# rafaelsoStanford/State_Policy_DiffusionModel

Hardware: AMD Instinct MI355X
Metric: denoise-steps/sec (B=4096, horizon=32) (higher is better)
Workload: dtype f32 (split-fp16 MFMA operands, fp32 accumulate)

## Files before the change

### state_policy_diffusionmodel_amd/csrc/device_utils.h

```cpp
#pragma once
#include <hip/hip_runtime.h>
#include "kernels.h"

namespace spdm {

__device__ __forceinline__ void sample_mean_rstd(const StatsRef& st, int b, float& mean, float& rstd) {
    const long long r0 = (long long)b * st.HW;
    const int first = (int)(r0 / st.m_tile);
    const int last = (int)((r0 + st.HW - 1) / st.m_tile);
    const int n = (last - first + 1) * st.n_tiles;
    const double* p = st.p + (size_t)b * st.slots * 2;
    double s1 = 0.0, s2 = 0.0;
    for (int i = 0; i < n; ++i) { s1 += p[2 * i]; s2 += p[2 * i + 1]; }
    const double m = s1 * st.inv_count;
    double var = s2 * st.inv_count - m * m;
    if (var < 0.0) var = 0.0;
    mean = (float)m;
    rstd = (float)(1.0 / sqrt(var + 1e-5));
}

__device__ __forceinline__ float sum_xor32(float v) {
    const unsigned u = __builtin_bit_cast(unsigned, v);
    const auto r = __builtin_amdgcn_permlane32_swap(u, u, false, false);
    return __builtin_bit_cast(float, (unsigned)r[0]) + __builtin_bit_cast(float, (unsigned)r[1]);
}
__device__ __forceinline__ float max_xor32(float v) {
    const unsigned u = __builtin_bit_cast(unsigned, v);
    const auto r = __builtin_amdgcn_permlane32_swap(u, u, false, false);
    return fmaxf(__builtin_bit_cast(float, (unsigned)r[0]), __builtin_bit_cast(float, (unsigned)r[1]));
}
__device__ __forceinline__ float sum_xor16(float v) {
    const unsigned u = __builtin_bit_cast(unsigned, v);
    const auto r = __builtin_amdgcn_permlane16_swap(u, u, false, false);
    return __builtin_bit_cast(float, (unsigned)r[0]) + __builtin_bit_cast(float, (unsigned)r[1]);
}
__device__ __forceinline__ double sum_xor32_f64(double v) {
    const unsigned long long u = __builtin_bit_cast(unsigned long long, v);
    const unsigned lo = (unsigned)u, hi = (unsigned)(u >> 32);
    const auto rl = __builtin_amdgcn_permlane32_swap(lo, lo, false, false);
    const auto rh = __builtin_amdgcn_permlane32_swap(hi, hi, false, false);
    const double a = __builtin_bit_cast(double, ((unsigned long long)(unsigned)rh[0] << 32) | (unsigned)rl[0]);
    const double b = __builtin_bit_cast(double, ((unsigned long long)(unsigned)rh[1] << 32) | (unsigned)rl[1]);
    return a + b;
// ... 154 lines not shown
```

### state_policy_diffusionmodel_amd/csrc/kernels.h

```cpp
#pragma once
#include <hip/hip_runtime.h>
#include <stdint.h>
#include <mutex>
#include <set>
#include <utility>
#include <vector>

namespace spdm {

inline hipError_t allow_full_lds(const void* kern) {
    static std::mutex mu;
    static std::set<std::pair<int, const void*>> done;
    int dev = 0;
    hipError_t e = hipGetDevice(&dev);
    if (e != hipSuccess) return e;
    std::lock_guard<std::mutex> lk(mu);
    if (done.count({dev, kern})) return hipSuccess;
    e = hipFuncSetAttribute(kern, hipFuncAttributeMaxDynamicSharedMemorySize, (int)(160 * 1024));
    if (e == hipSuccess) done.insert({dev, kern});
    return e;
}

struct StatsRef {
    const double* p;
// ... 2 lines not shown
    int n_tiles;
    int HW;
    double inv_count;
};

__host__ __device__ inline int stats_slots(int HW, int m_tile, int n_tiles) {
    return ((HW + m_tile - 2) / m_tile + 1) * n_tiles;
}

enum : unsigned {
    SW_NO_WIDE = 1u << 0, SW_NO_WIDE128 = 1u << 1, SW_NO_W2 = 1u << 2, SW_NO_T512 = 1u << 3, SW_T512 = 1u << 4,
    SW_T3_BIG = 1u << 5, SW_NO_SMALL_TPI3 = 1u << 6, SW_WIDE_N64_2X2 = 1u << 7, SW_NO_SA_FUSED = 1u << 8,
    SW_NO_SA_TAIL = 1u << 9, SW_ATTN_VALU = 1u << 10, SW_SA_NO_WLDS = 1u << 11, SW_NO_FILM_FOLD = 1u << 12,
    SW_NO_GRAPH = 1u << 13, SW_NO_SPLITK = 1u << 14, SW_ARENA_TRACE = 1u << 15, SW_NO_WIDE_PIPE = 1u << 16, SW_NO_SKINNY = 1u << 17, SW_DEEP = 1u << 18,
    SW_NO_FILM_LOCAL = 1u << 19, SW_NO_FUSED_SRC = 1u << 20, SW_FILM_LOCAL = 1u << 21, SW_PIN_GEOMETRY = 1u << 22, SW_NO_WP4 = 1u << 23, SW_G2 = 1u << 24, SW_NO_WP8 = 1u << 25, SW_NO_SA_HEAD = 1u << 26, SW_SA_HEAD = 1u << 27, SW_NO_REG64 = 1u << 28,
    SW_NO_SA_CROP = 1u << 29, SW_NO_SA_OUTC = 1u << 30,
};
struct SwitchName { const char* env; unsigned bit; };
inline const SwitchName* switch_table(int* n) {
    static const SwitchName t[] = {
        {"SPDM_NO_WIDE", SW_NO_WIDE}, {"SPDM_NO_WIDE128", SW_NO_WIDE128}, {"SPDM_NO_W2", SW_NO_W2}, {"SPDM_NO_T512", SW_NO_T512},
        {"SPDM_T512", SW_T512}, {"SPDM_T3_BIG", SW_T3_BIG}, {"SPDM_NO_SMALL_TPI3", SW_NO_SMALL_TPI3},
        {"SPDM_WIDE_N64_2X2", SW_WIDE_N64_2X2}, {"SPDM_NO_SA_FUSED", SW_NO_SA_FUSED}, {"SPDM_NO_SA_TAIL", SW_NO_SA_TAIL},
        {"SPDM_ATTN_VALU", SW_ATTN_VALU}, {"SPDM_SA_NO_WLDS", SW_SA_NO_WLDS}, {"SPDM_NO_FILM_FOLD", SW_NO_FILM_FOLD},
        {"SPDM_NO_GRAPH", SW_NO_GRAPH}, {"SPDM_NO_SPLITK", SW_NO_SPLITK}, {"SPDM_ARENA_TRACE", SW_ARENA_TRACE}, {"SPDM_NO_WIDE_PIPE", SW_NO_WIDE_PIPE}, {"SPDM_NO_SKINNY", SW_NO_SKINNY}, {"SPDM_DEEP", SW_DEEP},
        {"SPDM_NO_FILM_LOCAL", SW_NO_FILM_LOCAL}, {"SPDM_NO_FUSED_SRC", SW_NO_FUSED_SRC},
        {"SPDM_FILM_LOCAL", SW_FILM_LOCAL}, {"SPDM_PIN_GEOMETRY", SW_PIN_GEOMETRY},
        {"SPDM_NO_WP4", SW_NO_WP4}, {"SPDM_G2", SW_G2}, {"SPDM_NO_WP8", SW_NO_WP8},
        {"SPDM_NO_SA_HEAD", SW_NO_SA_HEAD}, {"SPDM_SA_HEAD", SW_SA_HEAD}, {"SPDM_NO_REG64", SW_NO_REG64},
        {"SPDM_NO_SA_CROP", SW_NO_SA_CROP}, {"SPDM_NO_SA_OUTC", SW_NO_SA_OUTC}};
    *n = (int)(sizeof(t) / sizeof(t[0]));
    return t;
}
unsigned switches_from_env();
int spdm_tune(int idx, int dflt);

enum { PRO_NONE = 0, PRO_GN = 1, PRO_GN_GELU = 2, PRO_POOL = 3, PRO_UPCAT = 4 };
enum { EPI_STATS = 0, EPI_BIAS = 1, EPI_BIAS_GELU = 2, EPI_BIAS_RESID = 3, EPI_PLAIN = 4 };

enum { ROUTE_GEMM = 0, ROUTE_SKINNY = 1, ROUTE_REG = 2, ROUTE_WIDE = 3 };
enum { VAR_PLAIN = 0, VAR_W2 = 1, VAR_WP4 = 2, VAR_WP8 = 3, VAR_PIPE = 4, VAR_G2 = 5 };
struct GemmRoute { int kernel, variant, m_tile, n_tile; };

struct GemmArgs {
    const float* src;  int src_ld;
// ... 154 lines not shown
struct SaCrop { int H0, D, Wp, lh, lw; const float* outc_w; float outc_b; float* eps; };
bool sa_crop_supported(int L, int C, int H0, int D);
hipError_t launch_sa_fused64(const float* x, float* out, int B, int L, const float* ln1_g, const float* ln1_b,
                             const float* ln2_g, const float* ln2_b, const void* const w_hl[8], const float* bqkv,
                             const float* bo, const float* b1, const float* b2, const float* ab, unsigned sw, hipStream_t s,
                             const FilmSpec* fs = nullptr, const SaCrop* crop = nullptr);

bool sa_tail_supported(int C, unsigned sw);
hipError_t launch_sa_tail(int C, const float* o, const float* x, float* out, int rows, const float* wf_o, const float* wf_1,
                          const float* wf_2, const float* b_o, const float* b_1, const float* b_2, const float* ln_g,
                          const float* ln_b, const float* ab, int L, hipStream_t s, const FilmSpec* fs = nullptr);
bool sa_tail_film_local(int C, int L);
bool sa_head_supported(int C, int L, unsigned sw);
hipError_t launch_sa_head(int C, const float* x, float* att, int rows, const float* wf_in, const float* b_in, const float* ln_g,
                          const float* ln_b, const float* ab, int L, hipStream_t s, const FilmSpec* fs = nullptr);
hipError_t launch_sa_qkv(int C, const float* x, float* qkv, int rows, const float* wf_in, const float* b_in, const float* ln_g,
                         const float* ln_b, const float* ab, int L, hipStream_t s, const FilmSpec* fs = nullptr);

}
```

### state_policy_diffusionmodel_amd/csrc/sa_tail.hip

```cpp
#include <algorithm>
#include <cstdlib>

#include "device_utils.h"

namespace spdm {

namespace {

typedef float tf32x4 __attribute__((ext_vector_type(4)));
typedef float tf32x2 __attribute__((ext_vector_type(2)));
typedef _Float16 tf16x8 __attribute__((ext_vector_type(8)));
typedef _Float16 tf16x2 __attribute__((ext_vector_type(2)));

constexpr float T_ACT_SCALE = 16.0f;
constexpr float T_DESCALE = 1.0f / 2048.0f;
constexpr int T_LDK = 36;
template <int C> struct TailShape {
    static_assert(C == 128 || C == 256, "C = 128 or 256");
    static constexpr int TM = 8192 / C;
    static constexpr int WM = TM / 32, WN = 4 / WM;
    static constexpr int NCH = C / 32;
    static constexpr int TPR = C / 4, RPP = 256 / TPR;
    static constexpr int NP = TM / RPP;
};

struct SaTailArgs {
    const float* o;
// ... 1 lines not shown
    float* out;
    int M;
    const float *wf_o, *wf_1, *wf_2;
    const float *b_o, *b_1, *b_2, *ln_g, *ln_b;
    const float* ab; int L;
    FilmSpec fs;
};

__device__ __forceinline__ tf32x2 tsplit2_plain(float a, float b) {
    const float xa = a * T_ACT_SCALE, xb = b * T_ACT_SCALE;
    const _Float16 ha = (_Float16)xa, hb = (_Float16)xb;
    const tf16x2 h = {ha, hb};
    const tf16x2 l = {(_Float16)(xa - (float)ha), (_Float16)(xb - (float)hb)};
    return tf32x2{__builtin_bit_cast(float, h), __builtin_bit_cast(float, l)};
}
#define TAIL_SPLIT2 tsplit2
__device__ __forceinline__ tf32x2 tsplit2(float a, float b) {
    unsigned h, l;
    split_pair_f16(a * T_ACT_SCALE, b * T_ACT_SCALE, h, l);
    return tf32x2{__builtin_bit_cast(float, h), __builtin_bit_cast(float, l)};
}
template <int TPR>
__device__ __forceinline__ float trow_sum(float v) {
    static_assert(TPR == 32 || TPR == 64, "rows of 32 or 64 lanes");
    v = sum_xor16(row16_sum_dpp(v));
    if (TPR == 64) v = sum_xor32(v);
    return v;
}

template <int C>
__device__ __forceinline__ void tail_film_fold(tf32x4 (&v)[8], const float* __restrict__ ab, int L, int m0, int M, int cq, int srow0) {
// ... 30 lines not shown
#pragma unroll
        for (int i = 0; i < 8; ++i) {
            const float* ab_ = abl + (size_t)(min(m0 + S::RPP * i + srow0, M - 1) / L - b_first) * 2 * C + cq * 4;
            v[i] = v[i] * *reinterpret_cast<const tf32x4*>(ab_) + *reinterpret_cast<const tf32x4*>(ab_ + C);
        }
    }
}

#ifdef SPDM_DIAG_TAIL
__device__ unsigned long long g_tail_stamps[64];
#define TAIL_STAMP(k_) if (blockIdx.x == 0 && threadIdx.x == 0) { asm volatile("s_waitcnt vmcnt(0) lgkmcnt(0)" ::: "memory"); g_tail_stamps[(C == 256 ? 16 : 0) + (k_)] = __builtin_amdgcn_s_memrealtime(); }
#else
#define TAIL_STAMP(k_)
#endif

template <int C>
__global__ __launch_bounds__(256, 2) void sa_tail_kernel(const SaTailArgs a) {
    TAIL_STAMP(0)
    using S = TailShape<C>;
    constexpr int T_C = C, T_M = S::TM, NCH = S::NCH, RPP = S::RPP, TPR = S::TPR;
    constexpr int RT = 2, CT = 4;
    constexpr int NP = S::NP;
    extern __shared__ __attribute__((aligned(16))) float smem[];
    const int tid = threadIdx.x, lane = tid & 63;
    const int wave = __builtin_amdgcn_readfirstlane(tid >> 6);
    const int wm = wave / S::WN, wn = wave % S::WN, l16 = lane & 15, kg = lane >> 4;
    const int M = a.M;
    const int m0 = blockIdx.x * T_M;

    float* Abuf = smem;
    float* otile = smem;

    const int c16 = tid % TPR, srow0 = tid / TPR;
    const int aoff0 = (wm * 32 + l16) * T_LDK + kg * 4;

    const size_t wlane = ((size_t)(wn * CT) * 2) * 256 + lane * 4;
    constexpr size_t WCHUNK = (size_t)(C / 16) * 2 * 256;
    tf16x8 fb[2][CT][2], fa[2][2];
#define TAIL_LOAD_B(slot_, w_, kc_)                                                                  \
    {                                                                                                \
        const float* p_ = (w_) + wlane + (size_t)(kc_) * WCHUNK;                                     \
        _Pragma("unroll") for (int c_ = 0; c_ < CT; ++c_) {                                         \
            fb[slot_][c_][0] = *reinterpret_cast<const tf16x8*>(p_ + c_ * 512);                      \
            fb[slot_][c_][1] = *reinterpret_cast<const tf16x8*>(p_ + c_ * 512 + 256);                \
        }                                                                                            \
    }
#define TAIL_LOAD_FA(slot_, kc_, rt_)                                                                \
    {                                                                                                \
        const float* p_ = Abuf + ((kc_) * T_M + (rt_) * 16) * T_LDK + aoff0;                         \
        fa[slot_][0] = *reinterpret_cast<const tf16x8*>(p_);                                         \
        fa[slot_][1] = *reinterpret_cast<const tf16x8*>(p_ + 16);                                    \
    }
#define TAIL_WRITE_SLAB(v_)                                                                          \
    _Pragma("unroll") for (int i_ = 0; i_ < NP; ++i_) {                                             \
        const tf32x2 p0_ = TAIL_SPLIT2(v_[i_].x, v_[i_].y), p1_ = TAIL_SPLIT2(v_[i_].z, v_[i_].w);   \
        float* rowp_ = Abuf + ((c16 >> 3) * T_M + RPP * i_ + srow0) * T_LDK;                         \
        *reinterpret_cast<tf32x2*>(rowp_ + (c16 & 7) * 2) = tf32x2{p0_.x, p1_.x};                    \
        *reinterpret_cast<tf32x2*>(rowp_ + 16 + (c16 & 7) * 2) = tf32x2{p0_.y, p1_.y};               \
    }
#define TAIL_GEMM(w_, wnext_)                                                                        \
    {                                                                                                \
        _Pragma("unroll") for (int rt_ = 0; rt_ < RT; ++rt_)                                        \
            _Pragma("unroll") for (int ct_ = 0; ct_ < CT; ++ct_) acc[rt_][ct_] = tf32x4{0.f, 0.f, 0.f, 0.f}; \
        TAIL_LOAD_FA(0, 0, 0)                                                                        \
        _Pragma("unroll") for (int kc = 0; kc < NCH; ++kc) {                                        \
            if (kc + 1 < NCH) { TAIL_LOAD_B((kc + 1) & 1, w_, kc + 1) } else { TAIL_LOAD_B(0, wnext_, 0) } \
            _Pragma("unroll") for (int rt = 0; rt < RT; ++rt) {                                     \
                if (rt + 1 < RT) { TAIL_LOAD_FA((rt + 1) & 1, kc, rt + 1) }                          \
                else if (kc + 1 < NCH) { TAIL_LOAD_FA(0, kc + 1, 0) }                                \
                __builtin_amdgcn_sched_barrier(0);                                                   \
// ... 16 lines not shown
                _Pragma("unroll") for (int j_ = 0; j_ < 4; ++j_)                                    \
                    otile[(wm * 32 + rt_ * 16 + 4 * kg + j_) * T_C + col_] = acc[rt_][ct_][j_] * T_DESCALE; \
            }                                                                                        \
        __syncthreads();                                                                             \
    }

    TAIL_LOAD_B(0, a.wf_o, 0)
    float* abl = smem + NCH * T_M * T_LDK;
    const tf32x4 bo = *reinterpret_cast<const tf32x4*>(a.b_o + c16 * 4);
    const tf32x4 g4 = *reinterpret_cast<const tf32x4*>(a.ln_g + c16 * 4);
    const tf32x4 b4 = *reinterpret_cast<const tf32x4*>(a.ln_b + c16 * 4);
    const tf32x4 b1 = *reinterpret_cast<const tf32x4*>(a.b_1 + c16 * 4);
    const tf32x4 b2 = *reinterpret_cast<const tf32x4*>(a.b_2 + c16 * 4);

    tf32x4 av[NP], v[NP];
#pragma unroll
    for (int i = 0; i < NP; ++i) {
        const int row = min(m0 + RPP * i + srow0, M - 1);
        v[i] = *reinterpret_cast<const tf32x4*>(a.o + (size_t)row * T_C + c16 * 4);
        if (m0 + RPP * i + srow0 >= M) v[i] = tf32x4{0.f, 0.f, 0.f, 0.f};
    }
    TAIL_WRITE_SLAB(v)
#pragma unroll
    for (int i = 0; i < NP; ++i) {
        const int row = min(m0 + RPP * i + srow0, M - 1);
        av[i] = *reinterpret_cast<const tf32x4*>(a.x + (size_t)row * T_C + c16 * 4);
    }
    if (a.ab != nullptr) tail_film_fold<C>(av, a.ab, a.L, m0, M, c16, srow0);
    if (a.fs.on) tail_film_rows<C>(a.fs, a.L, m0, M, wave, lane, abl);
    __syncthreads();
    if (a.fs.on) tail_film_fold_lds<C>(av, abl, a.L, m0, M, c16, srow0);
    TAIL_STAMP(1)

    tf32x4 acc[RT][CT];

    TAIL_GEMM(a.wf_o, a.wf_1)
    TAIL_STAMP(2)
    TAIL_ACC_TO_TILE()
    TAIL_STAMP(3)
    {
        float part[NP];
#pragma unroll
        for (int i = 0; i < NP; ++i) {
            const int r = RPP * i + srow0;
            tf32x4 t = *reinterpret_cast<const tf32x4*>(otile + r * T_C + c16 * 4);
            t += bo;
// ... 21 lines not shown
        for (int i = 0; i < NP; ++i) part[i] = row16_sum_dpp(part[i]);
#pragma unroll
        for (int i = 0; i < NP; ++i) part[i] = sum_xor16(part[i]);
        if (TPR == 64) {
#pragma unroll
            for (int i = 0; i < NP; ++i) part[i] = sum_xor32(part[i]);
        }
#pragma unroll
        for (int i = 0; i < NP; ++i) {
            const float rstd = __builtin_amdgcn_rsqf(part[i] * (1.0f / (float)C) + 1e-5f);
            const tf32x4 d = v[i];
            v[i] = tf32x4{d.x * rstd * g4.x + b4.x, d.y * rstd * g4.y + b4.y, d.z * rstd * g4.z + b4.z, d.w * rstd * g4.w + b4.w};
        }
    }
    __syncthreads();
    TAIL_WRITE_SLAB(v)
    __syncthreads();
    TAIL_STAMP(4)

    TAIL_GEMM(a.wf_1, a.wf_2)
    TAIL_STAMP(5)
    TAIL_ACC_TO_TILE()
    {
#pragma unroll
        for (int i = 0; i < NP; ++i) {
            tf32x4 t = *reinterpret_cast<const tf32x4*>(otile + (RPP * i + srow0) * T_C + c16 * 4);
            t += b1;
            v[i] = tf32x4{gelu_erf(t.x), gelu_erf(t.y), gelu_erf(t.z), gelu_erf(t.w)};
        }
    }
    __syncthreads();
    TAIL_WRITE_SLAB(v)
    __syncthreads();
    TAIL_STAMP(6)

    TAIL_GEMM(a.wf_2, a.wf_2)
    TAIL_STAMP(7)
    TAIL_ACC_TO_TILE()
    {
#pragma unroll
        for (int i = 0; i < NP; ++i) {
            const int r = RPP * i + srow0;
            if (m0 + r < M) {
                tf32x4 t = *reinterpret_cast<const tf32x4*>(otile + r * T_C + c16 * 4);
                t += b2;
                t += av[i];
                *reinterpret_cast<tf32x4*>(a.out + (size_t)(m0 + r) * T_C + c16 * 4) = t;
            }
        }
    }
    TAIL_STAMP(8)
}

struct SaQkvArgs {
    const float* x; float* qkv; int M;
    const float* wf;
    const float *b_in, *ln_g, *ln_b;
    const float* ab; int L;
    FilmSpec fs;
};

template <int C>
__global__ __launch_bounds__(256, 2) void sa_qkv_kernel(const SaQkvArgs a) {
    using S = TailShape<C>;
    constexpr int T_C = C, T_M = S::TM, NCH = S::NCH, RPP = S::RPP, TPR = S::TPR;
    constexpr int RT = 2, CT = 4;
// ... 53 lines not shown
#pragma unroll
        for (int i = 0; i < NP; ++i) part[i] = row16_sum_dpp(part[i]);
#pragma unroll
        for (int i = 0; i < NP; ++i) part[i] = sum_xor16(part[i]);
        if (TPR == 64) {
#pragma unroll
            for (int i = 0; i < NP; ++i) part[i] = sum_xor32(part[i]);
        }
#pragma unroll
        for (int i = 0; i < NP; ++i) {
            const float rstd = __builtin_amdgcn_rsqf(part[i] * (1.0f / (float)C) + 1e-5f);
            const tf32x4 d = v[i];
            v[i] = tf32x4{d.x * rstd * g4.x + b4.x, d.y * rstd * g4.y + b4.y, d.z * rstd * g4.z + b4.z, d.w * rstd * g4.w + b4.w};
        }
    }
    TAIL_WRITE_SLAB(v)
    __syncthreads();
    for (int g = g_lo; g < g_hi; ++g) {
        const float* wg = a.wf + (size_t)g * WPROD;
        const float* wnext = a.wf + (size_t)(g < 2 ? g + 1 : g) * WPROD;
        const tf32x4 bi = *reinterpret_cast<const tf32x4*>(a.b_in + g * T_C + c16 * 4);
        TAIL_GEMM(wg, wnext)
        {
            float* ot = smem + NCH * T_M * T_LDK;
            if (g > g_lo) __syncthreads();
#pragma unroll
            for (int rt_ = 0; rt_ < RT; ++rt_)
#pragma unroll
                for (int ct_ = 0; ct_ < CT; ++ct_) {
                    const int col_ = wn * 64 + ct_ * 16 + l16;
#pragma unroll
// ... 23 lines not shown
    FilmSpec fs;
};

__device__ __forceinline__ float row16_max_dpp(float v) {
#define DPP_MAX(ctrl_) v = fmaxf(v, __builtin_bit_cast(float, __builtin_amdgcn_update_dpp(0, __builtin_bit_cast(int, v), ctrl_, 0xf, 0xf, false)));
    DPP_MAX(0xB1) DPP_MAX(0x4E) DPP_MAX(0x141) DPP_MAX(0x140)
#undef DPP_MAX
    return v;
}
__device__ __forceinline__ float head_exp_neg(float x) {
    const float t = x * 1.44269504f;
    const float tl = __fmaf_rn(x, 1.44269504f, -t) + x * 1.925963033e-8f;
    return __builtin_amdgcn_exp2f(t) * (1.0f + tl * 0.69314718f);
}

#undef TAIL_SPLIT2
#define TAIL_SPLIT2 tsplit2_plain
template <int C>
__global__ __launch_bounds__(256, 2) void sa_head_kernel(const SaHeadArgs a) {
    using S = TailShape<C>;
    constexpr int T_C = C, T_M = S::TM, NCH = S::NCH, RPP = S::RPP, TPR = S::TPR;
    constexpr int NP = S::NP;
    constexpr int D = C / 4;
    constexpr int QROW = 2 * D + 8;
    constexpr int VROW = 2 * T_M + 8;
    constexpr int NKT = T_M / 16;
    constexpr int NDT = D / 16;
    static_assert(T_M * VROW <= 2 * T_M * QROW, "P aliases the q / k tiles");
    extern __shared__ __attribute__((aligned(16))) float smem[];
    const int tid = threadIdx.x, lane = tid & 63;
    const int wave = __builtin_amdgcn_readfirstlane(tid >> 6);
    const int l16 = lane & 15, kg = lane >> 4;
    const int M = a.M, L = a.L;
    const int m0 = blockIdx.x * T_M;
    float* Abuf = smem;
    _Float16* Qs = reinterpret_cast<_Float16*>(smem + NCH * T_M * T_LDK);
    _Float16* Ks = Qs + T_M * QROW;
    _Float16* Vt = Ks + T_M * QROW;
    _Float16* Ps = Qs;
    const int c16 = tid % TPR, srow0 = tid / TPR;

    {
        tf32x4 v[NP];
        const tf32x4 g4 = *reinterpret_cast<const tf32x4*>(a.ln_g + c16 * 4);
        const tf32x4 b4 = *reinterpret_cast<const tf32x4*>(a.ln_b + c16 * 4);
#pragma unroll
        for (int i = 0; i < NP; ++i) {
            const int row = min(m0 + RPP * i + srow0, M - 1);
            v[i] = *reinterpret_cast<const tf32x4*>(a.x + (size_t)row * T_C + c16 * 4);
        }
        if (a.ab != nullptr) tail_film_fold<C>(v, a.ab, a.L, m0, M, c16, srow0);
        if (a.fs.on) {
            float* abl = reinterpret_cast<float*>(Qs);
            tail_film_rows<C>(a.fs, a.L, m0, M, wave, lane, abl);
            __syncthreads();
            tail_film_fold_lds<C>(v, abl, a.L, m0, M, c16, srow0);
            __syncthreads();
        }
        float part[NP];
#pragma unroll
        for (int i = 0; i < NP; ++i) part[i] = (v[i].x + v[i].y) + (v[i].z + v[i].w);
#pragma unroll
        for (int i = 0; i < NP; ++i) part[i] = trow_sum<TPR>(part[i]);
#pragma unroll
        for (int i = 0; i < NP; ++i) {
            const float mean = part[i] * (1.0f / (float)C);
            const tf32x4 t = v[i];
            const tf32x4 d = {t.x - mean, t.y - mean, t.z - mean, t.w - mean};
            v[i] = d;
            part[i] = (d.x * d.x + d.y * d.y) + (d.z * d.z + d.w * d.w);
        }
#pragma unroll
        for (int i = 0; i < NP; ++i) part[i] = trow_sum<TPR>(part[i]);
#pragma unroll
        for (int i = 0; i < NP; ++i) {
            const float rstd = __builtin_amdgcn_rsqf(part[i] * (1.0f / (float)C) + 1e-5f);
            const tf32x4 d = v[i];
            v[i] = tf32x4{d.x * rstd * g4.x + b4.x, d.y * rstd * g4.y + b4.y, d.z * rstd * g4.z + b4.z, d.w * rstd * g4.w + b4.w};
        }
        TAIL_WRITE_SLAB(v)
    }
    __syncthreads();

    const int rtw = (C == 128) ? wave : (wave >> 1);
    const int cpw = (C == 128) ? 0 : (wave & 1);
    const bool attn_wave = wave < NKT;
    const float qscale = (D == 32) ? 0.17677669529663687f : 0.125f;
    constexpr size_t WCHUNK = (size_t)(3 * C / 16) * 2 * 256;

    tf16x8 fbw[2][2][2];
#define HEAD_WPTR(h_, g_) (a.wf + ((size_t)((g_) * (C / 16) + (h_) * (D / 16) + cpw * 2) * 2) * 256 + lane * 4)
#define HEAD_LOAD_W(slot_, wp_, kc_)                                                                 \
    _Pragma("unroll") for (int ct_ = 0; ct_ < 2; ++ct_) {                                           \
        fbw[slot_][ct_][0] = *reinterpret_cast<const tf16x8*>((wp_) + (size_t)(kc_) * WCHUNK + ct_ * 512);        \
        fbw[slot_][ct_][1] = *reinterpret_cast<const tf16x8*>((wp_) + (size_t)(kc_) * WCHUNK + ct_ * 512 + 256);  \
    }
    HEAD_LOAD_W(0, HEAD_WPTR(0, 0), 0)
    for (int h = 0; h < 4; ++h) {
#pragma unroll
        for (int g = 0; g < 3; ++g) {
            tf32x4 acc[2] = {tf32x4{0.f, 0.f, 0.f, 0.f}, tf32x4{0.f, 0.f, 0.f, 0.f}};
            const float* wp = HEAD_WPTR(h, g);
            const float* wnext = (g < 2) ? HEAD_WPTR(h, g + 1) : HEAD_WPTR(min(h + 1, 3), 0);
#pragma unroll
            for (int kc = 0; kc < NCH; ++kc) {
                if (kc + 1 < NCH) { HEAD_LOAD_W((kc + 1) & 1, wp, kc + 1) } else { HEAD_LOAD_W(0, wnext, 0) }
                const float* ap = Abuf + (kc * T_M + rtw * 16 + l16) * T_LDK + kg * 4;
                const tf16x8 a_h = *reinterpret_cast<const tf16x8*>(ap), a_l = *reinterpret_cast<const tf16x8*>(ap + 16);
#pragma unroll
                for (int ct = 0; ct < 2; ++ct) {
                    acc[ct] = __builtin_amdgcn_mfma_f32_16x16x32_f16(a_h, fbw[kc & 1][ct][0], acc[ct], 0, 0, 0);
                    acc[ct] = __builtin_amdgcn_mfma_f32_16x16x32_f16(a_h, fbw[kc & 1][ct][1], acc[ct], 0, 0, 0);
                    acc[ct] = __builtin_amdgcn_mfma_f32_16x16x32_f16(a_l, fbw[kc & 1][ct][0], acc[ct], 0, 0, 0);
                }
            }
#pragma unroll
            for (int ct = 0; ct < 2; ++ct) {
                const int col = cpw * 32 + ct * 16 + l16;
                const float bias = a.b_in[g * T_C + h * D + col];
#pragma unroll
                for (int j = 0; j < 4; ++j) {
                    const int row = rtw * 16 + 4 * kg + j;
                    float val = acc[ct][j] * T_DESCALE + bias;
                    if (g == 0) val *= qscale;
                    const float xs = val * T_ACT_SCALE;
                    const _Float16 hi = (_Float16)xs, lo = (_Float16)(xs - (float)hi);
                    if (g == 2) { Vt[col * VROW + row] = hi; Vt[col * VROW + T_M + row] = lo; }
                    else { _Float16* X = (g == 0) ? Qs : Ks; X[row * QROW + col] = hi; X[row * QROW + D + col] = lo; }
                }
            }
        }
        __syncthreads();

        tf32x4 sc[NKT];
#pragma unroll
        for (int kt = 0; kt < NKT; ++kt) sc[kt] = tf32x4{0.f, 0.f, 0.f, 0.f};
        if (attn_wave) {
#pragma unroll
            for (int ks = 0; ks < D / 32; ++ks) {
                const _Float16* qp = Qs + (wave * 16 + l16) * QROW + 32 * ks + 8 * kg;
                const tf16x8 q_h = *reinterpret_cast<const tf16x8*>(qp), q_l = *reinterpret_cast<const tf16x8*>(qp + D);
#pragma unroll
                for (int kt = 0; kt < NKT; ++kt) {
                    const _Float16* kp = Ks + (kt * 16 + l16) * QROW + 32 * ks + 8 * kg;
                    const tf16x8 k_h = *reinterpret_cast<const tf16x8*>(kp), k_l = *reinterpret_cast<const tf16x8*>(kp + D);
                    sc[kt] = __builtin_amdgcn_mfma_f32_16x16x32_f16(q_h, k_h, sc[kt], 0, 0, 0);
                    sc[kt] = __builtin_amdgcn_mfma_f32_16x16x32_f16(q_h, k_l, sc[kt], 0, 0, 0);
// ... 51 lines not shown
                    o[dt] = __builtin_amdgcn_mfma_f32_16x16x32_f16(p_h, v_h, o[dt], 0, 0, 0);
                    o[dt] = __builtin_amdgcn_mfma_f32_16x16x32_f16(p_h, v_l, o[dt], 0, 0, 0);
                    o[dt] = __builtin_amdgcn_mfma_f32_16x16x32_f16(p_l, v_h, o[dt], 0, 0, 0);
                }
            }
#pragma unroll
            for (int dt = 0; dt < NDT; ++dt)
#pragma unroll
                for (int j = 0; j < 4; ++j) {
                    const int row = m0 + wave * 16 + 4 * kg + j;
                    if (row < M) a.att[(size_t)row * T_C + h * D + dt * 16 + l16] = o[dt][j] * (1.0f / 16384.0f);
                }
        }
        __syncthreads();
    }
#undef TAIL_LOAD_B
#undef TAIL_LOAD_FA
#undef TAIL_WRITE_SLAB
#undef TAIL_GEMM
#undef TAIL_ACC_TO_TILE
}

}

#ifdef SPDM_DIAG_TAIL
extern "C" int spdm_debug_tail_stamps(unsigned long long* out64) {
    return hipMemcpyFromSymbol(out64, HIP_SYMBOL(g_tail_stamps), sizeof(unsigned long long) * 64) == hipSuccess ? 0 : -1;
}
#endif

bool sa_tail_supported(int C, unsigned sw) { return (C == 128 || C == 256) && !(sw & SW_NO_SA_TAIL); }

static int film_rows_cap(int TM, int L) { return (TM + L - 2) / L + 1; }
bool sa_tail_film_local(int C, int L) {
    if (!(C == 128 || C == 256) || L < 1) return false;
    return (size_t)film_rows_cap(8192 / C, L) * 2 * C * sizeof(float) <= (size_t)24 * 1024;
// ... 29 lines not shown
    if (fs && (ab || !sa_tail_film_local(C, L) || fs->C != C)) return hipErrorInvalidValue;
    SaHeadArgs a{};
    a.x = x; a.att = att; a.M = rows; a.wf = wf_in; a.b_in = b_in; a.ln_g = ln_g; a.ln_b = ln_b; a.ab = ab; a.L = L;
    if (fs) { a.fs = *fs; a.fs.on = 1; }
    const int TM = 8192 / C, D = C / 4;
    const size_t lds = (size_t)(C / 32) * TM * T_LDK * sizeof(float) + ((size_t)2 * TM * (2 * D + 8) + (size_t)D * (2 * TM + 8)) * sizeof(_Float16);
    if (fs && (size_t)film_rows_cap(TM, L) * 2 * C * sizeof(float) > ((size_t)2 * TM * (2 * D + 8) + (size_t)D * (2 * TM + 8)) * sizeof(_Float16)) return hipErrorInvalidValue;
    const void* kern = C == 128 ? reinterpret_cast<const void*>(sa_head_kernel<128>) : reinterpret_cast<const void*>(sa_head_kernel<256>);
    if (hipError_t e = allow_full_lds(kern); e != hipSuccess) return e;
    const int tiles = (rows + TM - 1) / TM;
    if (C == 128) hipLaunchKernelGGL(sa_head_kernel<128>, dim3(tiles), dim3(256), lds, s, a);
    else hipLaunchKernelGGL(sa_head_kernel<256>, dim3(tiles), dim3(256), lds, s, a);
    return hipGetLastError();
}

hipError_t launch_sa_qkv(int C, const float* x, float* qkv, int rows, const float* wf_in, const float* b_in, const float* ln_g,
                         const float* ln_b, const float* ab, int L, hipStream_t s, const FilmSpec* fs) {
    if (fs && (ab || L <= 0 || !sa_tail_film_local(C, L) || fs->C != C)) return hipErrorInvalidValue;
    if (rows <= 0 || (ab && L <= 0) || !x || !qkv || !wf_in || !b_in || !ln_g || !ln_b) return hipErrorInvalidValue;
    if (C != 128 && C != 256) return hipErrorInvalidValue;
    SaQkvArgs a{};
    a.x = x; a.qkv = qkv; a.M = rows; a.wf = wf_in; a.b_in = b_in; a.ln_g = ln_g; a.ln_b = ln_b; a.ab = ab; a.L = L;
    if (fs) { a.fs = *fs; a.fs.on = 1; }
    const int TM = 8192 / C;
    const size_t lds = (size_t)((C / 32) * TM * T_LDK + TM * C) * sizeof(float);
    const void* kern = C == 128 ? reinterpret_cast<const void*>(sa_qkv_kernel<128>) : reinterpret_cast<const void*>(sa_qkv_kernel<256>);
    if (hipError_t e = allow_full_lds(kern); e != hipSuccess) return e;
    const int tiles = (rows + TM - 1) / TM;
    const int gy = (tiles < spdm_tune(15, 512)) ? 3 : 1;
    if (C == 128) hipLaunchKernelGGL(sa_qkv_kernel<128>, dim3(tiles, gy), dim3(256), lds, s, a);
// ... 6 lines not shown
```

### state_policy_diffusionmodel_amd/csrc/spdm_api.hip

```cpp
#include <hip/hip_runtime.h>

#include <algorithm>
#include <cmath>
#include <cstdarg>
#include <cstdio>
#include <cstdlib>
#include <cstring>
#include <map>
#include <set>
#include <string>
#include <vector>

#include "../../include/spdm.h"
#include "kernels.h"

using namespace spdm;

static thread_local char g_err[512] = "";
static int fail(int code, const char* fmt, ...) {
    va_list ap;
    va_start(ap, fmt);
    vsnprintf(g_err, sizeof(g_err), fmt, ap);
    va_end(ap);
    return code;
// ... 1115 lines not shown
                eps_ready = true;
            }
            if (!err && !dry)
                check(launch_sa_fused64(x.p, out.p, B, L, w.ln_g, w.ln_b, w.ff_ln_g, w.ff_ln_b, w.fw, w.in_proj.b,
                                        w.out_proj.b, w.ff1.b, w.ff2.b, abp, h->sw, s, fs, cropped ? &crop : nullptr),
                      "fused attention block");
            free(x);
            free(xs);
            if (ab) free(*ab);
            return out;
        }
        Tensor qkv = ralloc(rows, 3 * C);
        const int TMh = 8192 / C;
        const bool head = h->split && sa_tail_supported(C, h->sw) && sa_head_supported(C, L, h->sw) && h->weights_loaded && w.qkv_wf &&
                          (!fs || sa_tail_film_local(C, L)) && ((Bg() * L + TMh - 1) / TMh) >= ((h->sw & SW_SA_HEAD) ? 1 : spdm_tune(16, 2048));
        if (!head) {
            if (h->split && sa_tail_supported(C, h->sw) && (!h->weights_loaded || w.qkv_wf)) {
                if (!err && !dry)
                    check(launch_sa_qkv(C, x.p, qkv.p, rows, w.qkv_wf, w.in_proj.b, w.ln_g, w.ln_b, abp, L, s, fs), "attention in_proj");
            } else {
                linear(x.p, C, rows, w.in_proj, qkv.p, EPI_BIAS, nullptr, &xs, w.ln_g, w.ln_b);
            }
        }
        free(xs);
        Tensor att = ralloc(rows, C);
        if (!err && !dry) {
            if (head) check(launch_sa_head(C, x.p, att.p, rows, w.qkv_wf, w.in_proj.b, w.ln_g, w.ln_b, abp, L, s, fs), "attention in_proj + core");
            else check(launch_attention_auto(qkv.p, att.p, B, L, C, 4, h->sw, s), "attention core");
        }
        free(qkv);
        if (h->split && sa_tail_supported(C, h->sw) && (!h->weights_loaded || w.tail_wf[0])) {
            Tensor out = talloc(C, level);
            if (!err && !dry)
                check(launch_sa_tail(C, att.p, x.p, out.p, rows, w.tail_wf[0], w.tail_wf[1], w.tail_wf[2], w.out_proj.b, w.ff1.b,
                                        w.ff2.b, w.ff_ln_g, w.ff_ln_b, abp, L, s, fs), "attention tail");
            free(att);
            free(x);
            if (ab) free(*ab);
            return out;
        }
        Tensor av = talloc(C, level);
        const int nt_av = gemm_geometry((rows / B) * Bg(), C, C, 1, 1, 1, (h->split && w.out_proj.ws) ? 1 : 0, h->sw).n_tiles;
        StatsBuf avs = row_stats_alloc(rows, C, nt_av);
        linear(att.p, C, rows, w.out_proj, av.p, EPI_BIAS_RESID, x.p, nullptr, nullptr, nullptr, avs.p);
        free(att);
        free(x);
        Tensor f1 = ralloc(rows, C);
        linear(av.p, C, rows, w.ff1, f1.p, EPI_BIAS_GELU, nullptr, &avs, w.ff_ln_g, w.ff_ln_b);
        free(avs);
        Tensor out = talloc(C, level);
// ... 1169 lines not shown
```

Before: 497,100.

## Fuse attention head and tail into one self-attention block kernel

Adds a sa_block kernel that runs the in_proj+attention head body and then the out_proj/FF tail body in one launch. The attention output is kept in registers and written into LDS as split fp16, and the residual input rows are passed in registers, so the att tensor no longer round-trips through global memory. The head loop is unrolled in block mode and attention uses a new per-head softmax path with permlane reductions. This enabled-by-default route costs extra registers (the per-head outputs held across heads), which may hurt occupancy or cause spills, in exchange for one fewer launch and less memory traffic.

After: 499,600, median of 6. About the same (+0.5%).

```diff
diff --git a/state_policy_diffusionmodel_amd/csrc/device_utils.h b/state_policy_diffusionmodel_amd/csrc/device_utils.h
--- a/state_policy_diffusionmodel_amd/csrc/device_utils.h
+++ b/state_policy_diffusionmodel_amd/csrc/device_utils.h
@@ -27,6 +27,11 @@
 __device__ __forceinline__ float max_xor32(float v) {
     const unsigned u = __builtin_bit_cast(unsigned, v);
     const auto r = __builtin_amdgcn_permlane32_swap(u, u, false, false);
+    return fmaxf(__builtin_bit_cast(float, (unsigned)r[0]), __builtin_bit_cast(float, (unsigned)r[1]));
+}
+__device__ __forceinline__ float max_xor16(float v) {
+    const unsigned u = __builtin_bit_cast(unsigned, v);
+    const auto r = __builtin_amdgcn_permlane16_swap(u, u, false, false);
     return fmaxf(__builtin_bit_cast(float, (unsigned)r[0]), __builtin_bit_cast(float, (unsigned)r[1]));
 }
 __device__ __forceinline__ float sum_xor16(float v) {
diff --git a/state_policy_diffusionmodel_amd/csrc/kernels.h b/state_policy_diffusionmodel_amd/csrc/kernels.h
--- a/state_policy_diffusionmodel_amd/csrc/kernels.h
+++ b/state_policy_diffusionmodel_amd/csrc/kernels.h
@@ -40,7 +40,7 @@
     SW_NO_SA_TAIL = 1u << 9, SW_ATTN_VALU = 1u << 10, SW_SA_NO_WLDS = 1u << 11, SW_NO_FILM_FOLD = 1u << 12,
     SW_NO_GRAPH = 1u << 13, SW_NO_SPLITK = 1u << 14, SW_ARENA_TRACE = 1u << 15, SW_NO_WIDE_PIPE = 1u << 16, SW_NO_SKINNY = 1u << 17, SW_DEEP = 1u << 18,
     SW_NO_FILM_LOCAL = 1u << 19, SW_NO_FUSED_SRC = 1u << 20, SW_FILM_LOCAL = 1u << 21, SW_PIN_GEOMETRY = 1u << 22, SW_NO_WP4 = 1u << 23, SW_G2 = 1u << 24, SW_NO_WP8 = 1u << 25, SW_NO_SA_HEAD = 1u << 26, SW_SA_HEAD = 1u << 27, SW_NO_REG64 = 1u << 28,
-    SW_NO_SA_CROP = 1u << 29, SW_NO_SA_OUTC = 1u << 30,
+    SW_NO_SA_CROP = 1u << 29, SW_NO_SA_OUTC = 1u << 30, SW_NO_SA_BLOCK = 1u << 31,
 };
 struct SwitchName { const char* env; unsigned bit; };
 inline const SwitchName* switch_table(int* n) {
@@ -54,7 +54,7 @@
         {"SPDM_FILM_LOCAL", SW_FILM_LOCAL}, {"SPDM_PIN_GEOMETRY", SW_PIN_GEOMETRY},
         {"SPDM_NO_WP4", SW_NO_WP4}, {"SPDM_G2", SW_G2}, {"SPDM_NO_WP8", SW_NO_WP8},
         {"SPDM_NO_SA_HEAD", SW_NO_SA_HEAD}, {"SPDM_SA_HEAD", SW_SA_HEAD}, {"SPDM_NO_REG64", SW_NO_REG64},
-        {"SPDM_NO_SA_CROP", SW_NO_SA_CROP}, {"SPDM_NO_SA_OUTC", SW_NO_SA_OUTC}};
+        {"SPDM_NO_SA_CROP", SW_NO_SA_CROP}, {"SPDM_NO_SA_OUTC", SW_NO_SA_OUTC}, {"SPDM_NO_SA_BLOCK", SW_NO_SA_BLOCK}};
     *n = (int)(sizeof(t) / sizeof(t[0]));
     return t;
 }
@@ -239,6 +239,10 @@
 bool sa_head_supported(int C, int L, unsigned sw);
 hipError_t launch_sa_head(int C, const float* x, float* att, int rows, const float* wf_in, const float* b_in, const float* ln_g,
                           const float* ln_b, const float* ab, int L, hipStream_t s, const FilmSpec* fs = nullptr);
+hipError_t launch_sa_block(int C, const float* x, float* out, int rows, const float* wf_in, const float* b_in, const float* ln_g,
+                           const float* ln_b, const float* wf_o, const float* wf_1, const float* wf_2, const float* b_o,
+                           const float* b_1, const float* b_2, const float* ff_ln_g, const float* ff_ln_b, const float* ab, int L,
+                           hipStream_t s, const FilmSpec* fs = nullptr);
 hipError_t launch_sa_qkv(int C, const float* x, float* qkv, int rows, const float* wf_in, const float* b_in, const float* ln_g,
                          const float* ln_b, const float* ab, int L, hipStream_t s, const FilmSpec* fs = nullptr);
 
diff --git a/state_policy_diffusionmodel_amd/csrc/sa_tail.hip b/state_policy_diffusionmodel_amd/csrc/sa_tail.hip
--- a/state_policy_diffusionmodel_amd/csrc/sa_tail.hip
+++ b/state_policy_diffusionmodel_amd/csrc/sa_tail.hip
@@ -11,6 +11,7 @@
 typedef float tf32x2 __attribute__((ext_vector_type(2)));
 typedef _Float16 tf16x8 __attribute__((ext_vector_type(8)));
 typedef _Float16 tf16x2 __attribute__((ext_vector_type(2)));
+typedef _Float16 tf16x4 __attribute__((ext_vector_type(4)));
 
 constexpr float T_ACT_SCALE = 16.0f;
 constexpr float T_DESCALE = 1.0f / 2048.0f;
@@ -42,7 +43,6 @@
     const tf16x2 l = {(_Float16)(xa - (float)ha), (_Float16)(xb - (float)hb)};
     return tf32x2{__builtin_bit_cast(float, h), __builtin_bit_cast(float, l)};
 }
-#define TAIL_SPLIT2 tsplit2
 __device__ __forceinline__ tf32x2 tsplit2(float a, float b) {
     unsigned h, l;
     split_pair_f16(a * T_ACT_SCALE, b * T_ACT_SCALE, h, l);
@@ -103,14 +103,14 @@
 #define TAIL_STAMP(k_)
 #endif
 
-template <int C>
-__global__ __launch_bounds__(256, 2) void sa_tail_kernel(const SaTailArgs a) {
+template <int C, bool BLOCK>
+__device__ __forceinline__ void sa_tail_body(const SaTailArgs& a, float* smem, const tf32x4 (&xr)[8], const tf32x4 (&ob)[4][C / 64]) {
     TAIL_STAMP(0)
     using S = TailShape<C>;
     constexpr int T_C = C, T_M = S::TM, NCH = S::NCH, RPP = S::RPP, TPR = S::TPR;
     constexpr int RT = 2, CT = 4;
     constexpr int NP = S::NP;
-    extern __shared__ __attribute__((aligned(16))) float smem[];
+    static_assert(NP == 8, "8 row pieces per thread");
     const int tid = threadIdx.x, lane = tid & 63;
     const int wave = __builtin_amdgcn_readfirstlane(tid >> 6);
     const int wm = wave / S::WN, wn = wave % S::WN, l16 = lane & 15, kg = lane >> 4;
@@ -140,9 +140,9 @@
         fa[slot_][0] = *reinterpret_cast<const tf16x8*>(p_);                                         \
         fa[slot_][1] = *reinterpret_cast<const tf16x8*>(p_ + 16);                                    \
     }
-#define TAIL_WRITE_SLAB(v_)                                                                          \
+#define TAIL_WRITE_SLAB(v_, split_)                                                                  \
     _Pragma("unroll") for (int i_ = 0; i_ < NP; ++i_) {                                             \
-        const tf32x2 p0_ = TAIL_SPLIT2(v_[i_].x, v_[i_].y), p1_ = TAIL_SPLIT2(v_[i_].z, v_[i_].w);   \
+        const tf32x2 p0_ = split_(v_[i_].x, v_[i_].y), p1_ = split_(v_[i_].z, v_[i_].w);             \
         float* rowp_ = Abuf + ((c16 >> 3) * T_M + RPP * i_ + srow0) * T_LDK;                         \
         *reinterpret_cast<tf32x2*>(rowp_ + (c16 & 7) * 2) = tf32x2{p0_.x, p1_.x};                    \
         *reinterpret_cast<tf32x2*>(rowp_ + 16 + (c16 & 7) * 2) = tf32x2{p0_.y, p1_.y};               \
@@ -189,13 +189,38 @@
     const tf32x4 b2 = *reinterpret_cast<const tf32x4*>(a.b_2 + c16 * 4);
 
     tf32x4 av[NP], v[NP];
+    if constexpr (BLOCK) {
+        constexpr int D = C / 4, NKT = T_M / 16;
+        _Float16* const Ah = reinterpret_cast<_Float16*>(Abuf);
+        if (wave < NKT) {
+#pragma unroll
+            for (int h = 0; h < 4; ++h)
+#pragma unroll
+                for (int dt = 0; dt < D / 16; ++dt) {
+                    const int row = wave * 16 + l16, col = h * D + dt * 16 + 4 * kg;
+                    tf16x4 hi, lo;
+#pragma unroll
+                    for (int j = 0; j < 4; ++j) {
+                        const float xs = (ob[h][dt][j] * (1.0f / 16384.0f)) * T_ACT_SCALE;
+                        hi[j] = (_Float16)xs;
+                        lo[j] = (_Float16)(xs - (float)hi[j]);
+                    }
+                    _Float16* const p = Ah + ((col >> 5) * T_M + row) * (2 * T_LDK) + (col & 31);
+                    *reinterpret_cast<tf16x4*>(p) = hi;
+                    *reinterpret_cast<tf16x4*>(p + 32) = lo;
+                }
+        }
+#pragma unroll
+        for (int i = 0; i < NP; ++i) av[i] = xr[i];
+        __syncthreads();
+    } else {
 #pragma unroll
     for (int i = 0; i < NP; ++i) {
         const int row = min(m0 + RPP * i + srow0, M - 1);
         v[i] = *reinterpret_cast<const tf32x4*>(a.o + (size_t)row * T_C + c16 * 4);
         if (m0 + RPP * i + srow0 >= M) v[i] = tf32x4{0.f, 0.f, 0.f, 0.f};
     }
-    TAIL_WRITE_SLAB(v)
+    TAIL_WRITE_SLAB(v, tsplit2)
 #pragma unroll
     for (int i = 0; i < NP; ++i) {
         const int row = min(m0 + RPP * i + srow0, M - 1);
@@ -205,6 +230,7 @@
     if (a.fs.on) tail_film_rows<C>(a.fs, a.L, m0, M, wave, lane, abl);
     __syncthreads();
     if (a.fs.on) tail_film_fold_lds<C>(av, abl, a.L, m0, M, c16, srow0);
+    }
     TAIL_STAMP(1)
 
     tf32x4 acc[RT][CT];
@@ -256,7 +282,7 @@
         }
     }
     __syncthreads();
-    TAIL_WRITE_SLAB(v)
+    TAIL_WRITE_SLAB(v, tsplit2)
     __syncthreads();
     TAIL_STAMP(4)
 
@@ -272,7 +298,7 @@
         }
     }
     __syncthreads();
-    TAIL_WRITE_SLAB(v)
+    TAIL_WRITE_SLAB(v, tsplit2)
     __syncthreads();
     TAIL_STAMP(6)
 
@@ -292,6 +318,13 @@
         }
     }
     TAIL_STAMP(8)
+}
+
+template <int C>
+__global__ __launch_bounds__(256, 2) void sa_tail_kernel(const SaTailArgs a) {
+    extern __shared__ __attribute__((aligned(16))) float smem[];
+    tf32x4 xr[8], ob[4][C / 64];
+    sa_tail_body<C, false>(a, smem, xr, ob);
 }
 
 struct SaQkvArgs {
@@ -375,7 +408,7 @@
             v[i] = tf32x4{d.x * rstd * g4.x + b4.x, d.y * rstd * g4.y + b4.y, d.z * rstd * g4.z + b4.z, d.w * rstd * g4.w + b4.w};
         }
     }
-    TAIL_WRITE_SLAB(v)
+    TAIL_WRITE_SLAB(v, tsplit2)
     __syncthreads();
     for (int g = g_lo; g < g_hi; ++g) {
         const float* wg = a.wf + (size_t)g * WPROD;
@@ -429,10 +462,8 @@
     return __builtin_amdgcn_exp2f(t) * (1.0f + tl * 0.69314718f);
 }
 
-#undef TAIL_SPLIT2
-#define TAIL_SPLIT2 tsplit2_plain
-template <int C>
-__global__ __launch_bounds__(256, 2) void sa_head_kernel(const SaHeadArgs a) {
+template <int C, bool BLOCK>
+__device__ __forceinline__ void sa_head_body(const SaHeadArgs& a, float* smem, tf32x4 (&xr)[8], tf32x4 (&ob)[4][C / 64]) {
     using S = TailShape<C>;
     constexpr int T_C = C, T_M = S::TM, NCH = S::NCH, RPP = S::RPP, TPR = S::TPR;
     constexpr int NP = S::NP;
@@ -442,7 +473,6 @@
     constexpr int NKT = T_M / 16;
     constexpr int NDT = D / 16;
     static_assert(T_M * VROW <= 2 * T_M * QROW, "P aliases the q / k tiles");
-    extern __shared__ __attribute__((aligned(16))) float smem[];
     const int tid = threadIdx.x, lane = tid & 63;
     const int wave = __builtin_amdgcn_readfirstlane(tid >> 6);
     const int l16 = lane & 15, kg = lane >> 4;
@@ -472,6 +502,10 @@
             tail_film_fold_lds<C>(v, abl, a.L, m0, M, c16, srow0);
             __syncthreads();
         }
+        if constexpr (BLOCK) {
+#pragma unroll
+            for (int i = 0; i < NP; ++i) xr[i] = v[i];
+        }
         float part[NP];
 #pragma unroll
         for (int i = 0; i < NP; ++i) part[i] = (v[i].x + v[i].y) + (v[i].z + v[i].w);
@@ -493,7 +527,7 @@
             const tf32x4 d = v[i];
             v[i] = tf32x4{d.x * rstd * g4.x + b4.x, d.y * rstd * g4.y + b4.y, d.z * rstd * g4.z + b4.z, d.w * rstd * g4.w + b4.w};
         }
-        TAIL_WRITE_SLAB(v)
+        TAIL_WRITE_SLAB(v, tsplit2_plain)
     }
     __syncthreads();
 
@@ -511,6 +545,8 @@
         fbw[slot_][ct_][1] = *reinterpret_cast<const tf16x8*>((wp_) + (size_t)(kc_) * WCHUNK + ct_ * 512 + 256);  \
     }
     HEAD_LOAD_W(0, HEAD_WPTR(0, 0), 0)
+    constexpr int HUNROLL = BLOCK ? 4 : 1;
+#pragma unroll HUNROLL
     for (int h = 0; h < 4; ++h) {
 #pragma unroll
         for (int g = 0; g < 3; ++g) {
@@ -540,12 +576,83 @@
                     if (g == 0) val *= qscale;
                     const float xs = val * T_ACT_SCALE;
                     const _Float16 hi = (_Float16)xs, lo = (_Float16)(xs - (float)hi);
-                    if (g == 2) { Vt[col * VROW + row] = hi; Vt[col * VROW + T_M + row] = lo; }
+                    if (g == 2) {
+                        const int vr = BLOCK ? ((row & ~31) | ((row & 12) << 1) | ((row & 16) >> 2) | (row & 3)) : row;
+                        Vt[col * VROW + vr] = hi;
+                        Vt[col * VROW + T_M + vr] = lo;
+                    }
                     else { _Float16* X = (g == 0) ? Qs : Ks; X[row * QROW + col] = hi; X[row * QROW + D + col] = lo; }
                 }
             }
         }
         __syncthreads();
+
+        if constexpr (BLOCK) {
+            if (attn_wave) {
+                tf32x4 sc[NKT];
+#pragma unroll
+                for (int kt = 0; kt < NKT; ++kt) sc[kt] = tf32x4{0.f, 0.f, 0.f, 0.f};
+#pragma unroll
+                for (int ks = 0; ks < D / 32; ++ks) {
+                    const _Float16* qp = Qs + (wave * 16 + l16) * QROW + 32 * ks + 8 * kg;
+                    const tf16x8 q_h = *reinterpret_cast<const tf16x8*>(qp), q_l = *reinterpret_cast<const tf16x8*>(qp + D);
+#pragma unroll
+                    for (int kt = 0; kt < NKT; ++kt) {
+                        const _Float16* kp = Ks + (kt * 16 + l16) * QROW + 32 * ks + 8 * kg;
+                        const tf16x8 k_h = *reinterpret_cast<const tf16x8*>(kp), k_l = *reinterpret_cast<const tf16x8*>(kp + D);
+                        sc[kt] = __builtin_amdgcn_mfma_f32_16x16x32_f16(k_h, q_h, sc[kt], 0, 0, 0);
+                        sc[kt] = __builtin_amdgcn_mfma_f32_16x16x32_f16(k_h, q_l, sc[kt], 0, 0, 0);
+                        sc[kt] = __builtin_amdgcn_mfma_f32_16x16x32_f16(k_l, q_h, sc[kt], 0, 0, 0);
+                    }
+                }
+                const int smp = (wave * 16 + l16) / L;
+                float mx = -3.0e38f;
+#pragma unroll
+                for (int kt = 0; kt < NKT; ++kt)
+#pragma unroll
+                    for (int j = 0; j < 4; ++j) {
+                        const bool own = ((kt * 16 + 4 * kg + j) / L) == smp;
+                        sc[kt][j] = own ? sc[kt][j] * (1.0f / 256.0f) : -3.0e38f;
+                        mx = fmaxf(mx, sc[kt][j]);
+                    }
+                mx = max_xor32(max_xor16(mx));
+                float sum = 0.f;
+#pragma unroll
+                for (int kt = 0; kt < NKT; ++kt)
+#pragma unroll
+                    for (int j = 0; j < 4; ++j) {
+                        sc[kt][j] = (sc[kt][j] > -1.0e38f) ? head_exp_neg(sc[kt][j] - mx) : 0.f;
+                        sum += sc[kt][j];
+                    }
+                sum = sum_xor32(sum_xor16(sum));
+                const float inv = 1024.0f / sum;
+                tf32x4 o[NDT];
+#pragma unroll
+                for (int dt = 0; dt < NDT; ++dt) o[dt] = tf32x4{0.f, 0.f, 0.f, 0.f};
+#pragma unroll
+                for (int ks = 0; ks < T_M / 32; ++ks) {
+                    tf16x8 p_h, p_l;
+#pragma unroll
+                    for (int e = 0; e < 8; ++e) {
+                        const float ps = sc[2 * ks + (e >> 2)][e & 3] * inv;
+                        p_h[e] = (_Float16)ps;
+                        p_l[e] = (_Float16)(ps - (float)p_h[e]);
+                    }
+#pragma unroll
+                    for (int dt = 0; dt < NDT; ++dt) {
+                        const _Float16* vp = Vt + (dt * 16 + l16) * VROW + 32 * ks + 8 * kg;
+                        const tf16x8 v_h = *reinterpret_cast<const tf16x8*>(vp), v_l = *reinterpret_cast<const tf16x8*>(vp + T_M);
+                        o[dt] = __builtin_amdgcn_mfma_f32_16x16x32_f16(v_h, p_h, o[dt], 0, 0, 0);
+                        o[dt] = __builtin_amdgcn_mfma_f32_16x16x32_f16(v_l, p_h, o[dt], 0, 0, 0);
+                        o[dt] = __builtin_amdgcn_mfma_f32_16x16x32_f16(v_h, p_l, o[dt], 0, 0, 0);
+                    }
+                }
+#pragma unroll
+                for (int dt = 0; dt < NDT; ++dt) ob[h][dt] = o[dt];
+            }
+            __syncthreads();
+            continue;
+        }
 
         tf32x4 sc[NKT];
 #pragma unroll
@@ -627,12 +734,29 @@
         }
         __syncthreads();
     }
+}
+
+template <int C>
+__global__ __launch_bounds__(256, 2) void sa_head_kernel(const SaHeadArgs a) {
+    extern __shared__ __attribute__((aligned(16))) float smem[];
+    tf32x4 xr[8], ob[4][C / 64];
+    sa_head_body<C, false>(a, smem, xr, ob);
+}
+
+struct SaBlockArgs { SaHeadArgs head; SaTailArgs tail; };
+
+template <int C>
+__global__ __launch_bounds__(256, 2) void sa_block_kernel(const SaBlockArgs a) {
+    extern __shared__ __attribute__((aligned(16))) float smem[];
+    tf32x4 xr[8], ob[4][C / 64];
+    sa_head_body<C, true>(a.head, smem, xr, ob);
+    sa_tail_body<C, true>(a.tail, smem, xr, ob);
+}
 #undef TAIL_LOAD_B
 #undef TAIL_LOAD_FA
 #undef TAIL_WRITE_SLAB
 #undef TAIL_GEMM
 #undef TAIL_ACC_TO_TILE
-}
 
 }
 
@@ -692,6 +816,32 @@
     return hipGetLastError();
 }
 
+hipError_t launch_sa_block(int C, const float* x, float* out, int rows, const float* wf_in, const float* b_in, const float* ln_g,
+                           const float* ln_b, const float* wf_o, const float* wf_1, const float* wf_2, const float* b_o,
+                           const float* b_1, const float* b_2, const float* ff_ln_g, const float* ff_ln_b, const float* ab, int L,
+                           hipStream_t s, const FilmSpec* fs) {
+    if (rows <= 0 || !x || !out || !wf_in || !b_in || !ln_g || !ln_b || !wf_o || !wf_1 || !wf_2 || !b_o || !b_1 || !b_2 ||
+        !ff_ln_g || !ff_ln_b || !sa_head_supported(C, L, 0) || rows % L != 0)
+        return hipErrorInvalidValue;
+    if (fs && (ab || !sa_tail_film_local(C, L) || fs->C != C)) return hipErrorInvalidValue;
+    SaBlockArgs a{};
+    a.head.x = x; a.head.att = nullptr; a.head.M = rows; a.head.wf = wf_in; a.head.b_in = b_in; a.head.ln_g = ln_g;
+    a.head.ln_b = ln_b; a.head.ab = ab; a.head.L = L;
+    if (fs) { a.head.fs = *fs; a.head.fs.on = 1; }
+    a.tail.out = out; a.tail.M = rows; a.tail.wf_o = wf_o; a.tail.wf_1 = wf_1; a.tail.wf_2 = wf_2;
+    a.tail.b_o = b_o; a.tail.b_1 = b_1; a.tail.b_2 = b_2; a.tail.ln_g = ff_ln_g; a.tail.ln_b = ff_ln_b; a.tail.L = L;
+    const int TM = 8192 / C, D = C / 4;
+    const size_t tiles_lds = ((size_t)2 * TM * (2 * D + 8) + (size_t)D * (2 * TM + 8)) * sizeof(_Float16);
+    const size_t lds = (size_t)(C / 32) * TM * T_LDK * sizeof(float) + tiles_lds;
+    if (fs && (size_t)film_rows_cap(TM, L) * 2 * C * sizeof(float) > tiles_lds) return hipErrorInvalidValue;
+    const void* kern = C == 128 ? reinterpret_cast<const void*>(sa_block_kernel<128>) : reinterpret_cast<const void*>(sa_block_kernel<256>);
+    if (hipError_t e = allow_full_lds(kern); e != hipSuccess) return e;
+    const int tiles = (rows + TM - 1) / TM;
+    if (C == 128) hipLaunchKernelGGL(sa_block_kernel<128>, dim3(tiles), dim3(256), lds, s, a);
+    else hipLaunchKernelGGL(sa_block_kernel<256>, dim3(tiles), dim3(256), lds, s, a);
+    return hipGetLastError();
+}
+
 hipError_t launch_sa_qkv(int C, const float* x, float* qkv, int rows, const float* wf_in, const float* b_in, const float* ln_g,
                          const float* ln_b, const float* ab, int L, hipStream_t s, const FilmSpec* fs) {
     if (fs && (ab || L <= 0 || !sa_tail_film_local(C, L) || fs->C != C)) return hipErrorInvalidValue;
diff --git a/state_policy_diffusionmodel_amd/csrc/spdm_api.hip b/state_policy_diffusionmodel_amd/csrc/spdm_api.hip
--- a/state_policy_diffusionmodel_amd/csrc/spdm_api.hip
+++ b/state_policy_diffusionmodel_amd/csrc/spdm_api.hip
@@ -1153,6 +1153,7 @@
         const int TMh = 8192 / C;
         const bool head = h->split && sa_tail_supported(C, h->sw) && sa_head_supported(C, L, h->sw) && h->weights_loaded && w.qkv_wf &&
                           (!fs || sa_tail_film_local(C, L)) && ((Bg() * L + TMh - 1) / TMh) >= ((h->sw & SW_SA_HEAD) ? 1 : spdm_tune(16, 2048));
+        const bool block = head && w.tail_wf[0] && !(h->sw & SW_NO_SA_BLOCK);
         if (!head) {
             if (h->split && sa_tail_supported(C, h->sw) && (!h->weights_loaded || w.qkv_wf)) {
                 if (!err && !dry)
@@ -1163,16 +1164,22 @@
         }
         free(xs);
         Tensor att = ralloc(rows, C);
-        if (!err && !dry) {
+        if (!err && !dry && !block) {
             if (head) check(launch_sa_head(C, x.p, att.p, rows, w.qkv_wf, w.in_proj.b, w.ln_g, w.ln_b, abp, L, s, fs), "attention in_proj + core");
             else check(launch_attention_auto(qkv.p, att.p, B, L, C, 4, h->sw, s), "attention core");
         }
         free(qkv);
         if (h->split && sa_tail_supported(C, h->sw) && (!h->weights_loaded || w.tail_wf[0])) {
             Tensor out = talloc(C, level);
-            if (!err && !dry)
-                check(launch_sa_tail(C, att.p, x.p, out.p, rows, w.tail_wf[0], w.tail_wf[1], w.tail_wf[2], w.out_proj.b, w.ff1.b,
-                                        w.ff2.b, w.ff_ln_g, w.ff_ln_b, abp, L, s, fs), "attention tail");
+            if (!err && !dry) {
+                if (block)
+                    check(launch_sa_block(C, x.p, out.p, rows, w.qkv_wf, w.in_proj.b, w.ln_g, w.ln_b, w.tail_wf[0], w.tail_wf[1],
+                                          w.tail_wf[2], w.out_proj.b, w.ff1.b, w.ff2.b, w.ff_ln_g, w.ff_ln_b, abp, L, s, fs),
+                          "attention block");
+                else
+                    check(launch_sa_tail(C, att.p, x.p, out.p, rows, w.tail_wf[0], w.tail_wf[1], w.tail_wf[2], w.out_proj.b, w.ff1.b,
+                                            w.ff2.b, w.ff_ln_g, w.ff_ln_b, abp, L, s, fs), "attention tail");
+            }
             free(att);
             free(x);
             if (ab) free(*ab);
```
